# GreatV/oar-ocr

Hardware: AMD Instinct MI355X
Metric: images/sec end-to-end PP-OCRv6 det+rec (higher is better)
Workload: dtype f32; 1 GPU; PP-OCRv6-tiny-class det+rec (synthetic-weight graphs: det 447089 params, rec 1135700 params, V=6906), batch=32 synthetic 960x960 pages per GPU, 40 text lines/page; timed region = u8 pages in pageable HOST memory -> oar_ocr_predict -> oar_ocr_decode -> sorted boxes + texts + scores on the host; image_batch_size=32, region_batch_size=256, parallelism=image-parallel x1

## Files before the change

oar_ocr_amd/build.py:

```python
from __future__ import annotations

import os
import subprocess
import sys
from concurrent.futures import ThreadPoolExecutor
from pathlib import Path

HERE = Path(__file__).resolve().parent
CSRC = HERE / "csrc"
LIBDIR = HERE / "lib"
LIB = LIBDIR / "libOarMi355x.so"
SOURCES = ["common.cc", "onnx_parse.cc", "engine.cc", "db_host.cc", "poly_host.cc", "pipeline.cc", "c_api.cc", "ctc_host.cc", "image_decode.cc", "image_misc_decode.cc", "jpeg_decode.cc", "layout.cc", "kernels.hip", "igemm.hip", "igemm_ws_1x1.hip", "igemm_ws_gen.hip", "igemm_ws_x6.hip", "igemm_os_x6.hip", "igemm_ws3.hip", "igemm_rs3_x6.hip", "prepost.hip", "contours.hip", "jpeg.hip", "layout.hip", "dsblock.hip", "dsblock_k3s1.hip", "dsblock_k3s2.hip", "dsblock_k5s1.hip", "dsblock_k5s2.hip", "dsblock_wa_a.hip", "dsblock_wa_b.hip", "dsblock_rs_k3s11.hip", "dsblock_rs_k3s21.hip", "dsblock_rs_k3s12.hip", "dsblock_rs_k3s22.hip", "dsblock_rs_dbg.hip", "dsblock_cs.hip", "dsblock_pc.hip", "dsblock_rs2.hip", "ctc_head_x6.hip", "chain.hip", "attention_x6.hip", "igemm_lk_x6.hip", "index_ops.hip", "sla_decode.hip", "formula_decode.hip", "window_attention.hip", "deformable_attention.hip", "relpos_attention.hip", "mha_attention.hip", "add_layernorm.hip"]
HIPCC = os.environ.get("HIPCC", "/opt/rocm/bin/hipcc")
FLAGS = ["--offload-arch=gfx950", "-O3", "-std=c++17", "-fPIC", "-ffp-contract=off", "-fno-fast-math",
         "-Wno-unused-result", "-Wno-pass-failed"]
if os.environ.get("OAR_DSB_ABLATIONS"):
    FLAGS.append("-DOAR_DSB_ABLATIONS")


def _stale(out: Path, deps) -> bool:
    if not out.exists():
        return True
    t = out.stat().st_mtime
    return any(Path(d).stat().st_mtime > t for d in deps)


def build_lib(force: bool = False, verbose: bool = False) -> Path:
    LIBDIR.mkdir(exist_ok=True)
    objdir = LIBDIR / "obj"
    objdir.mkdir(exist_ok=True)
    headers = list(CSRC.glob("*.h")) + list(CSRC.glob("*.inc")) + [HERE.parent / "include" / "oar_mi355x.h"]
    jobs = []
    for s in SOURCES:
        src = CSRC / s
        obj = objdir / (s.replace(".", "_") + ".o")
# ... 38 lines not shown
```

oar_ocr_amd/csrc/engine.cc:

```cpp
#include "engine.h"

#include "dsblock.h"

#include <algorithm>
#include <cmath>
#include <cstring>
#include <set>
#include <sstream>

namespace oar {

using k::Act;

static int64_t numel(const std::vector<int64_t>& d) {
    int64_t n = 1;
    for (auto v : d) n *= v;
    return n;
}

Engine::Engine(const uint8_t* onnx, size_t len, int device_id, hipStream_t caller_stream) : device_(device_id) {
    int ndev = 0;
    if (hipGetDeviceCount(&ndev) != hipSuccess || ndev <= 0)
        fail(OAR_DEVICE, "no HIP device visible: libOarMi355x has no CPU fallback");
    OAR_CHECK(device_id >= 0 && device_id < ndev, OAR_DEVICE, "device_id out of range");
// ... 2705 lines not shown
        auto it = E.dev_consts_.find(key);
        if (it != E.dev_consts_.end()) return it->second;
        int64_t K = transB ? B.dims[1] : B.dims[0], N = transB ? B.dims[0] : B.dims[1];
        std::vector<float> w((size_t)N * K, 0.f);
        for (int64_t kk = 0; kk < K; ++kk)
            for (int64_t nn = 0; nn < N; ++nn) w[(size_t)nn * K + kk] = transB ? B.f[nn * K + kk] : B.f[kk * N + nn];
        return E.upload_const(key, to_fragments(fmt, w, N, K));
    }

    void get_pads(const GNode& n, int64_t H, int64_t W, int64_t kh, int64_t kw, int64_t sh, int64_t sw, int64_t dh, int64_t dw,
                  int64_t& pt, int64_t& pl, int64_t& pb, int64_t& pr) {
        std::vector<int64_t> pads = n.ais("pads");
        pt = pl = pb = pr = 0;
        if (pads.size() == 4) { pt = pads[0]; pl = pads[1]; pb = pads[2]; pr = pads[3]; }
        std::string ap = n.as("auto_pad", "NOTSET");
        if (ap == "SAME_UPPER" || ap == "SAME_LOWER") {
            int64_t oh = (H + sh - 1) / sh, ow = (W + sw - 1) / sw;
            int64_t th = std::max<int64_t>((oh - 1) * sh + (kh - 1) * dh + 1 - H, 0), tw = std::max<int64_t>((ow - 1) * sw + (kw - 1) * dw + 1 - W, 0);
            if (ap == "SAME_UPPER") { pt = th / 2; pb = th - pt; pl = tw / 2; pr = tw - pl; }
            else { pb = th / 2; pt = th - pb; pr = tw / 2; pl = tw - pr; }
        }
    }

    void op_conv(const GNode& n) {
        if (n.in.size() > 3 && !n.in[3].empty()) {
            TInfo xg = get(n.in[0]), gt = get(n.in[3]);
            const TInfo& wg = get(n.in[1]);
            bool ok = xg.dims.size() == 4 && !xg.host_int && !gt.host_int && wg.ht && wg.ht->dims.size() == 4 && gt.loc.kind != Loc::NONE && n.residual.empty();
            if (ok) {
                const int64_t N = xg.dims[0], C = xg.dims[1], HW = xg.dims[2] * xg.dims[3];
                ok = numel(gt.dims) == N * C && gt.dims.size() >= 2 && gt.dims[0] == N && gt.dims[1] == C && wg.ht->dims[1] == C && C % 8 == 0 &&
                     k::conv_igemm_se_ok(N * HW, (int)C, (int)wg.ht->dims[0], (int)HW);
            }
            if (!ok) {
                GNode mul;
                mul.op = "Mul"; mul.in = {n.in[0], n.in[3]}; mul.out = {n.out[0] + "::se"};
                op_binary(mul, 2);
                GNode c2 = n;
                c2.in.resize(3);
                c2.in[0] = mul.out[0];
                op_conv(c2);
                return;
            }
        }
        PendingConcat msrc;
        {
// ... 24 lines not shown
        int64_t pt, pl, pb, pr;
        get_pads(n, H, Wd, kh, kw, sh, sw, dh, dw, pt, pl, pb, pr);
        int64_t Ho = (H + pt + pb - dh * (kh - 1) - 1) / sh + 1, Wo = (Wd + pl + pr - dw * (kw - 1) - 1) / sw + 1;
        if (x.u8_stem) {
            OAR_CHECK(g == 1 && Cin == 3 && kh * kw * 3 <= 128 && n.residual.empty(), OAR_INTERNAL, "run_stem on a graph whose first node is not an RGB stem");
            const float* sb = has_input(n, 2) ? get(n.in[2]).loc.cptr : nullptr;
            TInfo& ys = new_out(n.out[0], {N, Cout, Ho, Wo}, Layout::CLAST);
            k::ConvP sp{};
            sp.N = (int)N; sp.H = (int)H; sp.W = (int)Wd; sp.Cin = 3; sp.Ho = (int)Ho; sp.Wo = (int)Wo; sp.Cout = (int)Cout;
            sp.kh = (int)kh; sp.kw = (int)kw; sp.sh = (int)sh; sp.sw = (int)sw; sp.pt = (int)pt; sp.pl = (int)pl; sp.dh = (int)dh; sp.dw = (int)dw;
            sp.groups = 1; sp.act = n.act; sp.bias = sb; sp.y_ld = (int)Cout; sp.convt2x2 = 0;
            sp.w = conv_weight_direct(n, W);
            const Loc ysl = ys.loc;
            step([=](const RunCtx& c) {
                OAR_CHECK(c.stem != nullptr, OAR_INTERNAL, "stem plan run without pages");
                k::ConvP q = sp;
                q.y = c.mut(ysl);
                k::conv_smallcin_u8(c.s, q, *c.stem);
            }, 2.0 * N * Ho * Wo * Cout * 3 * kh * kw, 3.0 * N * H * Wd + 4.0 * N * Ho * Wo * Cout);
            return;
        }
        Loc xin = msrc.src.empty() ? to_clast_loc(x) : Loc();
        const float* bias = has_input(n, 2) ? get(n.in[2]).loc.cptr : nullptr;
        Loc res;
        int res_up = 0;
        if (!n.residual.empty()) {
            const char* up_env = getenv("OAR_FUSE_RES_UP");
            const bool up_on = !up_env || atoi(up_env) != 0;
            if (const PendingResize* pr = peek_pending(n.residual)) {
                const bool f32_tile = g == 1 && Cin % 4 == 0 && Cout % 4 == 0 &&
                                      k::igemm_weight_format((long)(N * Ho * Wo), (int)(kh * kw * Cin), (int)Cout, kh == 1 && kw == 1 && sh == 1 && sw == 1 && pt == 0 && pl == 0, (int)Cin) == k::IGEMM_W_K16;
                if (up_on && f32_tile && pr->fh > 1 && pr->fh == pr->fw && pr->N == N && pr->C == Cout && pr->Ho == Ho && pr->Wo == Wo && Ho % pr->fh == 0 && Wo % pr->fw == 0 &&
                    pr->H * pr->fh == Ho && pr->W * pr->fw == Wo && N * Ho * Wo < ((int64_t)1 << 31)) {
                    res = pr->xin;
                    res_up = pr->fh;
                    pending_resize.erase(n.residual);
                }
            }
        }
        if (!n.residual.empty() && res_up == 0) {
            TInfo r = get(n.residual);
            if (r.host_int || r.dims != std::vector<int64_t>{N, Cout, Ho, Wo}) {
                GNode pre = n;
                pre.residual.clear();
                pre.out[0] = n.out[0] + "::pre";
                op_conv(pre);
// ... 2642 lines not shown
```

oar_ocr_amd/csrc/igemm.hip:

```cpp
#include "igemm_dev.h"

namespace oar {
namespace k {

template <int NT, int PF, bool IS1X1>
__global__ __launch_bounds__(256, 2) void conv_igemm_kernel(IgemmP p) {
    const int lane = threadIdx.x & 63, wave = threadIdx.x >> 6;
    const int pl_ = lane & 15, g = lane >> 4;
    const long b = blockIdx.x;
    const int xcd = (int)(b & 7);
    const long slot = b >> 3;
    const int ntile = (int)(slot % p.ny);
    const long mtile = (long)xcd * p.mx_per_xcd + slot / p.ny;
    if (slot / p.ny >= p.mx_per_xcd) return;
    const long m0 = (mtile * 4 + wave) * (PF * 16);
    const int nf0 = ntile * NT;
    if (m0 >= p.M) return;

    long pix_base[PF];
    int ih0[PF], iw0[PF];
#pragma unroll
    for (int pf = 0; pf < PF; ++pf) {
        long m = min(m0 + pf * 16 + pl_, p.M - 1);
        if (IS1X1) {
// ... 205 lines not shown
    const int nfrag = (N + 15) / 16, KC = (K + 15) / 16;
    int NT = 1, best = 1 << 30;
    for (int t = 4; t >= 1; --t) { int padded = (nfrag + t - 1) / t * t; if (padded < best) { best = padded; NT = t; } }
    const long ny = (nfrag + NT - 1) / NT;
    const long wave_tile_passes = ((M + 15) / 16) * ((nfrag + 7) / 8);
    const bool ws_auto = (N >= ws_min_n && wave_tile_passes >= 4096) || (K >= 512 && M >= 262144);
    const bool ws = (N & 3) == 0 && KC >= 2 && ws_mode != 0 && (ws_mode == 1 || ws_auto);
    return !ws && ((M + 15) / 16) * ny <= small_max;
}
bool conv_igemm_se_ok(long M, int K, int N, int hw) {
    static const bool on = [] { const char* e = getenv("OAR_FUSE_SE_SCALE"); return !e || atoi(e) != 0; }();
    if (!on || hw <= 0) return false;
    if (igemm_weight_format(M, K, N, true) == IGEMM_W_K16) {
        const char* e = getenv("OAR_FUSE_SE_SCALE_SMALL");
        const bool small_se = !(e && e[0] == '0');
        return small_se && (K & 3) == 0 && (N & 3) == 0 && f32_1x1_goes_small(M, K, N);
    }
    if (igemm_weight_format(M, K, N, true) != IGEMM_W_X6) return false;
    const int nfrag = (N + 15) / 16, nt = ws_x6_tile(K, nfrag);
    if (nt == 0 || os_mode() == 2) return false;
    const int ny = (nfrag + nt - 1) / nt;
    const size_t lds = (size_t)nt * ((K + 31) / 32) * 3072 + (size_t)nt * 64 + 16 + (size_t)ws_x6_se_rows(M, ny, hw) * K * 4;
    return lds <= 160 * 1024;
}

void conv_igemm(hipStream_t s, const ConvP& c) {
    IgemmP p;
    p.x = c.x; p.w = c.w; p.bias = c.bias; p.res = c.residual; p.y = c.y;
    p.H = c.H; p.W = c.W; p.Cin = c.Cin; p.kh = c.kh; p.kw = c.kw; p.sh = c.sh; p.sw = c.sw;
    p.pt = c.pt; p.pl = c.pl; p.dh = c.dh; p.dw = c.dw; p.y_ld = c.y_ld;
    p.act = c.act.kind; p.alpha = c.act.alpha; p.beta = c.act.beta;
    p.convt = c.convt2x2; p.Cout = c.Cout;
    p.ctc_part = c.ctc_part; p.ctc_valid = c.ctc_valid;
    p.se = c.se; p.se_hw = c.Ho * c.Wo;
    p.x_ld = c.x_ld > 0 ? c.x_ld : c.Cin; p.accum = c.accum;
    p.n_msrc = c.n_msrc;
    for (int i = 0; i < 8; ++i) { p.msrc[i] = i < c.n_msrc ? c.msrc[i] : nullptr; p.msrc_c[i] = i < c.n_msrc ? c.msrc_c[i] : 0; }
    p.res_up = c.residual ? c.res_up : 0;
    if (c.convt2x2) {
        p.Ho = c.H; p.Wo = c.W;
        p.M = (long)c.N * c.H * c.W; p.K = c.Cin; p.gemm_cout = 4 * c.Cout;
    } else {
        p.Ho = c.Ho; p.Wo = c.Wo;
        p.M = (long)c.N * c.Ho * c.Wo; p.K = c.kh * c.kw * c.Cin; p.gemm_cout = c.Cout;
    }
    const bool x6 = c.w_fmt == IGEMM_W_X6;
// ... 134 lines not shown
```

oar_ocr_amd/csrc/igemm_dev.h:

```cpp
#pragma once
#include <hip/hip_runtime.h>

#include <algorithm>
#include <cstdio>
#include <cstdlib>
#include <type_traits>
#include <vector>

#include "common.h"
#include "kernels_dev.h"

namespace oar {
namespace k {

struct IgemmP {
    const float* x;
    const float* w;
    const float* bias;
    const float* res;
    float* y;
    long M;
    int K, KC;
    int gemm_cout;
    int Cout;
// ... 169 lines not shown
        float4* dst = reinterpret_cast<float4*>(p.ctc_part) + row * ny + ntile;
        *dst = make_float4(m, sum, __int_as_float(last), 0.f);
    }
}

template <int NT, int PF>
__device__ __forceinline__ bool igemm_init_acc(const IgemmP& p, f32x4 (&acc)[NT][PF], int g, int nf0) {
    const bool fast = p.bias != nullptr && ((p.Cout & 3) == 0) && ((p.y_ld & 3) == 0);
#pragma clang loop unroll(full)
    for (int nf = 0; nf < NT; ++nf) {
        float4 b = make_float4(0.f, 0.f, 0.f, 0.f);
        if (fast) {
            const int c = (nf0 + nf) * 16 + g * 4;
            const int cc = c < p.gemm_cout ? c : 0;
            const int co = p.convt ? cc % p.Cout : cc;
            b = *reinterpret_cast<const float4*>(p.bias + co);
        }
#pragma clang loop unroll(full)
        for (int pf = 0; pf < PF; ++pf) acc[nf][pf] = (f32x4){b.x, b.y, b.z, b.w};
    }
    return fast;
}

void conv_igemm_ws_1x1(hipStream_t s, const IgemmP& p, int ws_nt, int ny, size_t lds);
void conv_igemm_ws_gen(hipStream_t s, const IgemmP& p, int ws_nt, int ny, size_t lds);
void conv_igemm_ws_x6(hipStream_t s, const IgemmP& p, int ws_nt, int ny, size_t lds);
int igemm_os_x6_tile(int nfrag);
void conv_igemm_os_x6(hipStream_t s, const IgemmP& p, int nfrag, bool is1x1);
bool conv_igemm_ws3_eligible(const IgemmP& p, int nfrag);
void conv_igemm_ws3(hipStream_t s, const IgemmP& p, int nfrag);
bool conv3x3_n16_x6_eligible(long M, int Cin, int Cout, long img_px, int y_ld);
std::vector<int> conv3x3_n16_x6_slices(long M, int Cin, int Cout, long img_px, int y_ld);
void conv_lk_x6(hipStream_t s, const IgemmP& p, int n_images);
void conv3x3_n16_x6(hipStream_t s, const IgemmP& p, int n_images);

}
}
```

oar_ocr_amd/csrc/igemm_ws_x6.hip:

```cpp
#include "igemm_dev.h"

namespace oar {
namespace k {

typedef __bf16 bf16x8 __attribute__((ext_vector_type(8)));

struct IgemmWsX6P {
    IgemmP g;
    int ny;
    int groups;
    long wt_per_xcd;
    long wt_total;
    int se_cap;
};

__device__ __forceinline__ void split3(const f32x4& a, const f32x4& b, uint4& h, uint4& m, uint4& l) {
    const float f[8] = {a[0], a[1], a[2], a[3], b[0], b[1], b[2], b[3]};
    unsigned hh[8], mm[8], ll[8];
#pragma clang loop unroll(full)
    for (int e = 0; e < 8; ++e) {
        const unsigned u = __float_as_uint(f[e]);
        const unsigned uh = u & 0xFFFF0000u;
        const float r1 = f[e] - __uint_as_float(uh);
        const unsigned um = __float_as_uint(r1) & 0xFFFF0000u;
        const float r2 = r1 - __uint_as_float(um);
        hh[e] = uh; mm[e] = um; ll[e] = __float_as_uint(r2) & 0xFFFF0000u;
    }
    h = make_uint4((hh[0] >> 16) | hh[1], (hh[2] >> 16) | hh[3], (hh[4] >> 16) | hh[5], (hh[6] >> 16) | hh[7]);
    m = make_uint4((mm[0] >> 16) | mm[1], (mm[2] >> 16) | mm[3], (mm[4] >> 16) | mm[5], (mm[6] >> 16) | mm[7]);
    l = make_uint4((ll[0] >> 16) | ll[1], (ll[2] >> 16) | ll[3], (ll[4] >> 16) | ll[5], (ll[6] >> 16) | ll[7]);
}

template <int NT, bool CTC = false, bool SE = false, int PF = 1>
__global__ __launch_bounds__(PF == 2 ? 512 : 1024) void conv_igemm_ws_x6_kernel(IgemmWsX6P q) {
    extern __shared__ uint4 wx_lds[];
    const IgemmP& p = q.g;
    const int lane = threadIdx.x & 63;
    const int pl_ = lane & 15, g = lane >> 4;
    const int xcd = (int)(blockIdx.x & 7);
    const int j = (int)(blockIdx.x >> 3);
    const int per_xcd = (int)(gridDim.x >> 3);
    const int team = j % q.groups, member = j / q.groups, team_size = (per_xcd - team + q.groups - 1) / q.groups;
    float* lds_bias = reinterpret_cast<float*>(wx_lds + (long)NT * p.KC * 3 * 64);
    unsigned* ws_ctr = reinterpret_cast<unsigned*>(lds_bias + NT * 16);
    float* se_lds = reinterpret_cast<float*>(ws_ctr + 4);
    long wt_begin, wt_count;
    {
        const long x0 = (long)xcd * q.wt_per_xcd, x1 = min(q.wt_total, x0 + q.wt_per_xcd);
        const long n_x = max(0L, x1 - x0), share = (n_x + team_size - 1) / team_size;
        wt_begin = x0 + (long)member * share;
        wt_count = max(0L, min(share, x1 - wt_begin));
    }
    int se_first = 0;
    if (SE && wt_count > 0) {
// ... 169 lines not shown
            m0 = m0n; u = un;
#pragma clang loop unroll(full)
            for (int pf = 0; pf < PF; ++pf) cur_row[pf] = nxt_row[pf];
        }
        asm volatile("s_waitcnt vmcnt(0)" ::: "memory");
        tie(s0); tie(s1); tie(s2);
    }
}

static int ws_x6_se_rows_pf(long M, int ny, int hw, int pf) {
    const int per_xcd = 32;
    const long wt_total = (M + 16 * pf - 1) / (16 * pf), wt_per_xcd = (wt_total + 7) / 8;
    const int groups = ny < per_xcd ? ny : per_xcd, team_min = per_xcd / groups;
    const long share = (wt_per_xcd + team_min - 1) / team_min;
    return (int)((share * 16 * pf + hw - 1) / hw) + 1;
}
static int ws_x6_pf(long M, bool ctc, int act) {
    static const int force = [] { const char* e = getenv("OAR_WS_X6_PF"); return e ? atoi(e) : 0; }();
    if (ctc) return 1;
    if (force == 1 || force == 2) return force;
    const bool cheap = act == ACT_NONE || act == ACT_RELU || act == ACT_HSWISH || act == ACT_HSIGMOID || act == ACT_LEAKY || act == ACT_CLIP;
    return (cheap && M >= 98304) ? 2 : 1;
}
int ws_x6_se_rows(long M, int ny, int hw) { return std::max(ws_x6_se_rows_pf(M, ny, hw, 1), ws_x6_se_rows_pf(M, ny, hw, 2)); }

template <int NT, bool CTC = false, bool SE = false, int PF = 1>
static void launch_ws_x6(hipStream_t s, const IgemmP& p, int ny, size_t lds) {
    OAR_MAX_LDS_ONCE((conv_igemm_ws_x6_kernel<NT, CTC, SE, PF>), 160 * 1024);
    IgemmWsX6P q;
    q.g = p; q.ny = ny;
    const int per_xcd = 32;
    q.wt_total = (p.M + 16 * PF - 1) / (16 * PF);
    q.wt_per_xcd = (q.wt_total + 7) / 8;
    q.groups = ny < per_xcd ? ny : per_xcd;
    q.se_cap = 0;
    if (SE) {
        q.se_cap = ws_x6_se_rows_pf(p.M, ny, p.se_hw, PF);
        lds += (size_t)q.se_cap * p.K * 4;
        OAR_CHECK(lds <= 160 * 1024, OAR_INTERNAL, "conv_igemm_ws_x6: the gate rows do not fit LDS (conv_igemm_se_ok should have said no)");
    }
    hipLaunchKernelGGL((conv_igemm_ws_x6_kernel<NT, CTC, SE, PF>), dim3(per_xcd * 8), dim3(PF == 2 ? 512 : 1024), lds, s, q);
}

void conv_igemm_ws_x6(hipStream_t s, const IgemmP& p, int ws_nt, int ny, size_t lds) {
    if (p.ctc_part) { launch_ws_x6<8, true>(s, p, ny, lds); return; }
    const bool two = ws_x6_pf(p.M, false, p.act) == 2;
// ... 18 lines not shown
```

oar_ocr_amd/csrc/kernels.h:

```cpp
#pragma once
#include <hip/hip_runtime.h>

#include <cstdint>
#include <vector>

namespace oar {
namespace k {

enum ActKind : int { ACT_NONE = 0, ACT_RELU, ACT_HSWISH, ACT_HSIGMOID, ACT_SIGMOID, ACT_SWISH, ACT_LEAKY, ACT_CLIP, ACT_TANH, ACT_GELU_ERF,
                     ACT_ERF, ACT_SQRT, ACT_EXP, ACT_ABS, ACT_NEG, ACT_RECIP, ACT_LOG, ACT_GELU_TANH, ACT_SOFTPLUS, ACT_FLOOR, ACT_CEIL, ACT_ROUND, ACT_NOT };
struct Act {
    int kind = ACT_NONE;
    float alpha = 0.f, beta = 0.f;
};

struct ConvP {
    int N, H, W, Cin;
    int Ho, Wo, Cout;
    int kh, kw, sh, sw, pt, pl, dh, dw, groups;
    Act act;
    const float* x;
    const float* w;
    const float* bias;
    const float* residual;
// ... 1 lines not shown
    int y_ld;
    int convt2x2;
    int w_fmt;
    float* ctc_part;
    int ctc_valid;
    const float* se;
    int res_up;
    int n_msrc;
    const float* msrc[8];
    int msrc_c[8];
    int accum;
    int x_ld;
    float* gap_part;
};
enum : int { IGEMM_W_K16 = 0, IGEMM_W_X6 = 1, IGEMM_W_X6RS = 2, IGEMM_W_X6CS = 3 };

void conv_igemm(hipStream_t s, const ConvP& p);
int igemm_weight_format(long M, int K, int N, bool is1x1, int Cin = 0, long same3x3_px = 0, bool lk_ok = false);
bool conv_lk_x6_eligible(int kh, int kw, int sh, int sw, int pt, int pl, int dh, int dw, int H, int W, int Ho, int Wo, int Cin, int Cout, int y_ld, long M);
bool conv_grouped_x6_ok(long M, int K, int N, int Cin);
bool conv_msrc_ok(long M, int K, int N);
std::vector<int> conv3x3_n16_slices(long M, int Cin, int Cout, long img_px, int y_ld);
bool conv_igemm_se_ok(long M, int K, int N, int hw);
void conv_dw(hipStream_t s, const ConvP& p);
int conv_dw_gap_tiles(const ConvP& p);
void global_avgpool_finish(hipStream_t s, const float* part, float* y, int N, int tiles, int C, int hw);
void conv_direct(hipStream_t s, const ConvP& p);
struct StemImg { const uint8_t* ptr; int32_t w; int32_t pad; };
struct StemU8 { const uint8_t* pages[32]; int src[3]; float alpha[3], beta[3]; const StemImg* dev = nullptr; };
void conv_smallcin_u8(hipStream_t s, const ConvP& p, const StemU8& st);
struct ConvT2Pair {
    const float* x; float* y;
    const float *w1, *b1, *w2, *b2;
    int N, H, W, C0, C1, C2;
    Act act1, act2;
};
bool convt2x2_pair_supported(int C0, int C1, int C2);
void convt2x2_pair(hipStream_t s, const ConvT2Pair& p);
void convt_direct(hipStream_t s, const ConvP& p);

struct PoolP {
    int N, H, W, C, Ho, Wo, kh, kw, sh, sw, pt, pl;
    int pb, pr;
    int is_max, count_include_pad;
    const float* x;
    float* y;
// ... 197 lines not shown
```

oar_ocr_amd/csrc/pipeline.cc:

```cpp
#include "pipeline.h"

#include <algorithm>
#include <map>
#include <string>
#include <cmath>
#include <chrono>
#include <cstdlib>
#include <cstring>
#include <sched.h>

namespace oar {

namespace {
struct PhaseTimer {
    bool on;
    std::chrono::steady_clock::time_point t0;
    std::vector<std::pair<const char*, double>> marks;
    PhaseTimer() {
        static const bool en = [] { const char* e = getenv("OAR_TIMING"); return e && (e[0] == '1' || e[0] == '2'); }();
        on = en;
        t0 = std::chrono::steady_clock::now();
    }
    void mark(const char* name) {
        if (!on) return;
// ... 1197 lines not shown
        for (auto& c : b) { ws.push_back(c.w); hs.push_back(c.h); }
        std::vector<int32_t> rws;
        Wts[bi] = host::rec_tensor_width(ws, hs, img_h, img_w, (int)cfg_.max_img_w, rws);
        const Plan& probe = eng_->plan_for({(int64_t)b.size(), 3, img_h, Wts[bi]}, true, false, nullptr, fuse_stem);
        OAR_CHECK(!probe.outputs.empty(), OAR_INTERNAL, "CRNN: no output returned from inference");
        fuse_tail[bi] = probe.outputs[0].dims.size() == 3 && probe.outputs[0].dims[2] > 1024;
        const Plan& plan = fuse_tail[bi] ? eng_->plan_for({(int64_t)b.size(), 3, img_h, Wts[bi]}, true, true, nullptr, fuse_stem) : probe;
        const PlanOutput& po = plan.outputs[0];
        OAR_CHECK(po.dims.size() == 3, OAR_SHAPE_MISMATCH, "CRNN: expected 3D output (batch, time, vocab)");
        OAR_CHECK(po.dims[0] == (int64_t)b.size(), OAR_SHAPE_MISMATCH, "CRNN: output batch differs from input batch");
        outs[bi].T = (uint32_t)po.dims[1]; outs[bi].V = (uint32_t)po.dims[2]; outs[bi].Wt = (uint32_t)Wts[bi];
        pend[bi].row0 = row_total; pend[bi].rows = (size_t)b.size() * po.dims[1];
        if (po.dims[2] == 0) pend[bi].rows = 0;
        row_total += pend[bi].rows;
    }
    if (row_total * 8 > idx_dev_.cap || row_total * 4 > prob_dev_.cap) {
        OAR_HIP(hipStreamSynchronize(s));
        idx_dev_.reserve(row_total * 8); prob_dev_.reserve(row_total * 4);
    }
    idx_host_.reserve(row_total * 8); prob_host_.reserve(row_total * 4);
    const int n_lanes = 1 + (int)lanes_.size();
    std::vector<char> lane_used(n_lanes, 0);
    int next_lane = 0;
    for (size_t bi = 0; bi < batches.size(); ++bi) {
        const auto& b = batches[bi];
        if (b.empty()) continue;
        const int lane = next_lane;
        next_lane = (next_lane + 1) % n_lanes;
        lane_used[lane] = 1;
        Engine& eng = lane_engine(lane);
        hipStream_t sl = eng.stream();
        int Wt = 0;
        const float* in = nullptr;
        const pp::ResizedImg* imgs = nullptr;
        if (fuse_stem) imgs = pack_u8(b, Wt, desc_slot, stage_slot, lane);
        else in = pack(b, Wt, false, desc_slot, stage_slot, lane);
        desc_slot += b.size();
        for (auto& c : b) if (!c.dev) stage_slot += ((size_t)c.w * c.h * 3 + 63) & ~(size_t)63;
        k::StemU8 st{};
        if (fuse_stem) {
            st.src[0] = 2; st.src[1] = 1; st.src[2] = 0;
            st.dev = reinterpret_cast<const k::StemImg*>(imgs);
        }
        const Plan& plan = fuse_stem ? eng.run_stem(st, {(int64_t)b.size(), 3, img_h, Wt}, fuse_tail[bi] != 0)
                                     : eng.run(in, {(int64_t)b.size(), 3, img_h, Wt}, true, fuse_tail[bi] != 0);
        if (pend[bi].rows == 0) continue;
        const PlanOutput& po = plan.outputs[0];
        if (plan.skipped_softmax && plan.ctc_part.kind != Loc::NONE)
            k::ctc_combine(sl, eng.out_ptr(plan.ctc_part), (int64_t)pend[bi].rows, plan.ctc_tiles, idx_dev_.as<int64_t>() + pend[bi].row0,
// ... 556 lines not shown
```

Before: 2458 images/sec.

## Fuse 1x1 conv with trailing height-average pool and schedule smallest rec batch first

Adds a new kernel that computes a 1x1 pointwise conv (optionally SE-gated) via split-bf16 MFMA and reduces it directly into an AveragePool over full height and width-2 windows. This avoids writing and re-reading the full conv output. The planner only uses it behind an opt-in env var. Separately, the recognizer batch loop now moves the smallest batch to the front when several lanes exist, so lanes start work sooner. The fused kernel adds a large new code path with atomic work-stealing and its own numerics.

Result: faster. 2509 images/sec (median of 6 runs) (+2.1%).

```diff
diff --git a/oar_ocr_amd/build.py b/oar_ocr_amd/build.py
--- a/oar_ocr_amd/build.py
+++ b/oar_ocr_amd/build.py
@@ -10,7 +10,7 @@
 CSRC = HERE / "csrc"
 LIBDIR = HERE / "lib"
 LIB = LIBDIR / "libOarMi355x.so"
-SOURCES = ["common.cc", "onnx_parse.cc", "engine.cc", "db_host.cc", "poly_host.cc", "pipeline.cc", "c_api.cc", "ctc_host.cc", "image_decode.cc", "image_misc_decode.cc", "jpeg_decode.cc", "layout.cc", "kernels.hip", "igemm.hip", "igemm_ws_1x1.hip", "igemm_ws_gen.hip", "igemm_ws_x6.hip", "igemm_os_x6.hip", "igemm_ws3.hip", "igemm_rs3_x6.hip", "prepost.hip", "contours.hip", "jpeg.hip", "layout.hip", "dsblock.hip", "dsblock_k3s1.hip", "dsblock_k3s2.hip", "dsblock_k5s1.hip", "dsblock_k5s2.hip", "dsblock_wa_a.hip", "dsblock_wa_b.hip", "dsblock_rs_k3s11.hip", "dsblock_rs_k3s21.hip", "dsblock_rs_k3s12.hip", "dsblock_rs_k3s22.hip", "dsblock_rs_dbg.hip", "dsblock_cs.hip", "dsblock_pc.hip", "dsblock_rs2.hip", "ctc_head_x6.hip", "chain.hip", "attention_x6.hip", "igemm_lk_x6.hip", "index_ops.hip", "sla_decode.hip", "formula_decode.hip", "window_attention.hip", "deformable_attention.hip", "relpos_attention.hip", "mha_attention.hip", "add_layernorm.hip"]
+SOURCES = ["common.cc", "onnx_parse.cc", "engine.cc", "db_host.cc", "poly_host.cc", "pipeline.cc", "c_api.cc", "ctc_host.cc", "image_decode.cc", "image_misc_decode.cc", "jpeg_decode.cc", "layout.cc", "kernels.hip", "igemm.hip", "igemm_ws_1x1.hip", "igemm_ws_gen.hip", "igemm_ws_x6.hip", "igemm_os_x6.hip", "igemm_ws3.hip", "igemm_rs3_x6.hip", "prepost.hip", "contours.hip", "jpeg.hip", "layout.hip", "dsblock.hip", "dsblock_k3s1.hip", "dsblock_k3s2.hip", "dsblock_k5s1.hip", "dsblock_k5s2.hip", "dsblock_wa_a.hip", "dsblock_wa_b.hip", "dsblock_rs_k3s11.hip", "dsblock_rs_k3s21.hip", "dsblock_rs_k3s12.hip", "dsblock_rs_k3s22.hip", "dsblock_rs_dbg.hip", "dsblock_cs.hip", "dsblock_pc.hip", "dsblock_rs2.hip", "ctc_head_x6.hip", "chain.hip", "attention_x6.hip", "igemm_lk_x6.hip", "index_ops.hip", "sla_decode.hip", "formula_decode.hip", "window_attention.hip", "deformable_attention.hip", "relpos_attention.hip", "mha_attention.hip", "add_layernorm.hip", "se_tail.hip"]
 HIPCC = os.environ.get("HIPCC", "/opt/rocm/bin/hipcc")
 FLAGS = ["--offload-arch=gfx950", "-O3", "-std=c++17", "-fPIC", "-ffp-contract=off", "-fno-fast-math",
          "-Wno-unused-result", "-Wno-pass-failed"]
diff --git a/oar_ocr_amd/csrc/engine.cc b/oar_ocr_amd/csrc/engine.cc
--- a/oar_ocr_amd/csrc/engine.cc
+++ b/oar_ocr_amd/csrc/engine.cc
@@ -2751,6 +2751,44 @@
         }
     }
 
+    bool try_conv_pool(const GNode& n, const TInfo& x, const HostTensor& W, const Loc& xin, const float* bias) {
+        const char* fe = getenv("OAR_FUSE_SE_TAIL");
+        if (!(fe && atoi(fe) != 0) || cur + 1 >= (int)E.nodes_.size() || n.out.size() != 1 || !n.residual.empty()) return false;
+        const GNode& pn = E.nodes_[cur + 1];
+        if (pn.op != "AveragePool" || pn.in.size() != 1 || pn.in[0] != n.out[0] || pn.out.size() != 1 || pn.ai("ceil_mode", 0) != 0) return false;
+        for (auto& o : E.output_names_) if (o == n.out[0]) return false;
+        for (int j = 0; j < (int)E.nodes_.size(); ++j) {
+            const GNode& q = E.nodes_[j];
+            if (j != cur + 1) for (auto& s : q.in) if (s == n.out[0]) return false;
+            if (q.residual == n.out[0]) return false;
+        }
+        const int64_t N = x.dims[0], Cin = x.dims[1], H = x.dims[2], Wd = x.dims[3], Cout = W.dims[0];
+        auto ks = pn.ais("kernel_shape"), st = pn.ais("strides");
+        if (ks.size() != 2 || st.size() != 2 || ks[0] != H || ks[1] != 2 || st[1] != 2 || Wd < 2) return false;
+        int64_t pt, pl, pb, pr;
+        get_pads(pn, H, Wd, ks[0], ks[1], st[0], st[1], 1, 1, pt, pl, pb, pr);
+        if (pt || pl || pb || pr) return false;
+        const bool gated = has_input(n, 3);
+        if (N * H * Wd >= ((int64_t)1 << 31) || !k::conv1x1_pool_ok((int)N, (int)H, (int)Wd, (int)Cin, (int)Cout, gated, n.act.kind)) return false;
+        const int64_t T = Wd / 2;
+        Loc gate;
+        if (gated) gate = get(n.in[3]).loc;
+        TInfo& y = new_out(pn.out[0], {N, Cout, 1, T}, Layout::CLAST);
+        k::ConvP p{};
+        p.N = (int)N; p.H = (int)H; p.W = (int)Wd; p.Cin = (int)Cin; p.Ho = 1; p.Wo = (int)T; p.Cout = (int)Cout;
+        p.kh = 1; p.kw = 1; p.sh = 1; p.sw = 1; p.dh = 1; p.dw = 1; p.groups = 1; p.act = n.act; p.bias = bias; p.y_ld = (int)Cout;
+        p.w_fmt = k::IGEMM_W_X6;
+        p.w = conv_weight_igemm(n, W, p.w_fmt);
+        const Loc yl = y.loc;
+        step([=](const RunCtx& c) {
+            k::ConvP q = p;
+            q.x = c.at(xin); q.y = c.mut(yl); q.se = gated ? c.at(gate) : nullptr;
+            k::conv1x1_pool(c.s, q);
+        }, 2.0 * N * H * Wd * Cout * Cin, 4.0 * (N * H * Wd * Cin + N * T * Cout + numel(W.dims)));
+        fused_into_prev.insert(cur + 1);
+        return true;
+    }
+
     void op_conv(const GNode& n) {
         if (n.in.size() > 3 && !n.in[3].empty()) {
             TInfo xg = get(n.in[0]), gt = get(n.in[3]);
@@ -2821,6 +2859,7 @@
         }
         Loc xin = msrc.src.empty() ? to_clast_loc(x) : Loc();
         const float* bias = has_input(n, 2) ? get(n.in[2]).loc.cptr : nullptr;
+        if (msrc.src.empty() && g == 1 && kh == 1 && kw == 1 && sh == 1 && sw == 1 && pt == 0 && pl == 0 && pb == 0 && pr == 0 && try_conv_pool(n, x, W, xin, bias)) return;
         Loc res;
         int res_up = 0;
         if (!n.residual.empty()) {
diff --git a/oar_ocr_amd/csrc/igemm.hip b/oar_ocr_amd/csrc/igemm.hip
--- a/oar_ocr_amd/csrc/igemm.hip
+++ b/oar_ocr_amd/csrc/igemm.hip
@@ -251,6 +251,17 @@
     const int ny = (nfrag + nt - 1) / nt;
     const size_t lds = (size_t)nt * ((K + 31) / 32) * 3072 + (size_t)nt * 64 + 16 + (size_t)ws_x6_se_rows(M, ny, hw) * K * 4;
     return lds <= 160 * 1024;
+}
+
+int conv_igemm_ws_x6_tile(long M, int K, int N, int Cin, bool gated, int hw, int act) {
+    if ((N & 3) || igemm_weight_format(M, K, N, true, Cin) != IGEMM_W_X6) return 0;
+    const int nfrag = (N + 15) / 16, nt = ws_x6_tile(K, nfrag);
+    if (nt == 0 || os_mode() == 2) return 0;
+    if (gated) return conv_igemm_se_ok(M, K, N, hw) ? nt : 0;
+    static const bool os_wide = [] { const char* e = getenv("OAR_IGEMM_OS_WIDE"); return !e || atoi(e) != 0; }();
+    const bool cheap_act = act == ACT_NONE || act == ACT_RELU;
+    if (os_wide && os_mode() != 0 && cheap_act && K >= 320 && N >= 512 && nt <= 4 && os_x6_eligible(M, K, N, Cin)) return 0;
+    return nt;
 }
 
 void conv_igemm(hipStream_t s, const ConvP& c) {
diff --git a/oar_ocr_amd/csrc/igemm_dev.h b/oar_ocr_amd/csrc/igemm_dev.h
--- a/oar_ocr_amd/csrc/igemm_dev.h
+++ b/oar_ocr_amd/csrc/igemm_dev.h
@@ -215,6 +215,24 @@
     return fast;
 }
 
+typedef __bf16 bf16x8 __attribute__((ext_vector_type(8)));
+__device__ __forceinline__ void split3(const f32x4& a, const f32x4& b, uint4& h, uint4& m, uint4& l) {
+    const float f[8] = {a[0], a[1], a[2], a[3], b[0], b[1], b[2], b[3]};
+    unsigned hh[8], mm[8], ll[8];
+#pragma clang loop unroll(full)
+    for (int e = 0; e < 8; ++e) {
+        const unsigned u = __float_as_uint(f[e]);
+        const unsigned uh = u & 0xFFFF0000u;
+        const float r1 = f[e] - __uint_as_float(uh);
+        const unsigned um = __float_as_uint(r1) & 0xFFFF0000u;
+        const float r2 = r1 - __uint_as_float(um);
+        hh[e] = uh; mm[e] = um; ll[e] = __float_as_uint(r2) & 0xFFFF0000u;
+    }
+    h = make_uint4((hh[0] >> 16) | hh[1], (hh[2] >> 16) | hh[3], (hh[4] >> 16) | hh[5], (hh[6] >> 16) | hh[7]);
+    m = make_uint4((mm[0] >> 16) | mm[1], (mm[2] >> 16) | mm[3], (mm[4] >> 16) | mm[5], (mm[6] >> 16) | mm[7]);
+    l = make_uint4((ll[0] >> 16) | ll[1], (ll[2] >> 16) | ll[3], (ll[4] >> 16) | ll[5], (ll[6] >> 16) | ll[7]);
+}
+
 void conv_igemm_ws_1x1(hipStream_t s, const IgemmP& p, int ws_nt, int ny, size_t lds);
 void conv_igemm_ws_gen(hipStream_t s, const IgemmP& p, int ws_nt, int ny, size_t lds);
 void conv_igemm_ws_x6(hipStream_t s, const IgemmP& p, int ws_nt, int ny, size_t lds);
diff --git a/oar_ocr_amd/csrc/igemm_ws_x6.hip b/oar_ocr_amd/csrc/igemm_ws_x6.hip
--- a/oar_ocr_amd/csrc/igemm_ws_x6.hip
+++ b/oar_ocr_amd/csrc/igemm_ws_x6.hip
@@ -2,8 +2,6 @@
 
 namespace oar {
 namespace k {
-
-typedef __bf16 bf16x8 __attribute__((ext_vector_type(8)));
 
 struct IgemmWsX6P {
     IgemmP g;
@@ -13,23 +11,6 @@
     long wt_total;
     int se_cap;
 };
-
-__device__ __forceinline__ void split3(const f32x4& a, const f32x4& b, uint4& h, uint4& m, uint4& l) {
-    const float f[8] = {a[0], a[1], a[2], a[3], b[0], b[1], b[2], b[3]};
-    unsigned hh[8], mm[8], ll[8];
-#pragma clang loop unroll(full)
-    for (int e = 0; e < 8; ++e) {
-        const unsigned u = __float_as_uint(f[e]);
-        const unsigned uh = u & 0xFFFF0000u;
-        const float r1 = f[e] - __uint_as_float(uh);
-        const unsigned um = __float_as_uint(r1) & 0xFFFF0000u;
-        const float r2 = r1 - __uint_as_float(um);
-        hh[e] = uh; mm[e] = um; ll[e] = __float_as_uint(r2) & 0xFFFF0000u;
-    }
-    h = make_uint4((hh[0] >> 16) | hh[1], (hh[2] >> 16) | hh[3], (hh[4] >> 16) | hh[5], (hh[6] >> 16) | hh[7]);
-    m = make_uint4((mm[0] >> 16) | mm[1], (mm[2] >> 16) | mm[3], (mm[4] >> 16) | mm[5], (mm[6] >> 16) | mm[7]);
-    l = make_uint4((ll[0] >> 16) | ll[1], (ll[2] >> 16) | ll[3], (ll[4] >> 16) | ll[5], (ll[6] >> 16) | ll[7]);
-}
 
 template <int NT, bool CTC = false, bool SE = false, int PF = 1>
 __global__ __launch_bounds__(PF == 2 ? 512 : 1024) void conv_igemm_ws_x6_kernel(IgemmWsX6P q) {
@@ -245,6 +226,7 @@
     const bool cheap = act == ACT_NONE || act == ACT_RELU || act == ACT_HSWISH || act == ACT_HSIGMOID || act == ACT_LEAKY || act == ACT_CLIP;
     return (cheap && M >= 98304) ? 2 : 1;
 }
+int ws_x6_pixel_frags(long M, int act) { return ws_x6_pf(M, false, act); }
 int ws_x6_se_rows(long M, int ny, int hw) { return std::max(ws_x6_se_rows_pf(M, ny, hw, 1), ws_x6_se_rows_pf(M, ny, hw, 2)); }
 
 template <int NT, bool CTC = false, bool SE = false, int PF = 1>
diff --git a/oar_ocr_amd/csrc/kernels.h b/oar_ocr_amd/csrc/kernels.h
--- a/oar_ocr_amd/csrc/kernels.h
+++ b/oar_ocr_amd/csrc/kernels.h
@@ -47,6 +47,8 @@
 bool conv_msrc_ok(long M, int K, int N);
 std::vector<int> conv3x3_n16_slices(long M, int Cin, int Cout, long img_px, int y_ld);
 bool conv_igemm_se_ok(long M, int K, int N, int hw);
+bool conv1x1_pool_ok(int N, int H, int W, int Cin, int Cout, bool gated, int act);
+void conv1x1_pool(hipStream_t s, const ConvP& p);
 void conv_dw(hipStream_t s, const ConvP& p);
 int conv_dw_gap_tiles(const ConvP& p);
 void global_avgpool_finish(hipStream_t s, const float* part, float* y, int N, int tiles, int C, int hw);
diff --git a/oar_ocr_amd/csrc/pipeline.cc b/oar_ocr_amd/csrc/pipeline.cc
--- a/oar_ocr_amd/csrc/pipeline.cc
+++ b/oar_ocr_amd/csrc/pipeline.cc
@@ -1243,9 +1243,18 @@
     const int n_lanes = 1 + (int)lanes_.size();
     std::vector<char> lane_used(n_lanes, 0);
     int next_lane = 0;
-    for (size_t bi = 0; bi < batches.size(); ++bi) {
+    std::vector<size_t> order;
+    for (size_t bi = 0; bi < batches.size(); ++bi) if (!batches[bi].empty()) order.push_back(bi);
+    {
+        const char* e = getenv("OAR_REC_SHORT_FIRST");
+        if (!(e && atoi(e) == 0) && n_lanes > 1 && order.size() > 2) {
+            size_t best = 0;
+            for (size_t i = 1; i < order.size(); ++i) if (batches[order[i]].size() < batches[order[best]].size()) best = i;
+            std::rotate(order.begin(), order.begin() + (ptrdiff_t)best, order.begin() + (ptrdiff_t)best + 1);
+        }
+    }
+    for (size_t bi : order) {
         const auto& b = batches[bi];
-        if (b.empty()) continue;
         const int lane = next_lane;
         next_lane = (next_lane + 1) % n_lanes;
         lane_used[lane] = 1;
diff --git a/oar_ocr_amd/csrc/se_tail.hip b/oar_ocr_amd/csrc/se_tail.hip
--- /dev/null
+++ b/oar_ocr_amd/csrc/se_tail.hip
@@ -0,0 +1,324 @@
+#include "igemm_dev.h"
+
+namespace oar {
+namespace k {
+
+int conv_igemm_ws_x6_tile(long M, int K, int N, int Cin, bool gated, int hw, int act);
+int ws_x6_pixel_frags(long M, int act);
+
+namespace {
+
+struct PwPoolP {
+    IgemmP g;
+    int ny;
+    int groups;
+    long wt_per_xcd;
+    long wt_total;
+    int se_cap;
+    int cb;
+    int T;
+};
+
+constexpr int kPoolThreads = 512;
+
+template <int NT, bool SE, int PF>
+__global__ __launch_bounds__(kPoolThreads) void conv1x1_pool_x6_kernel(PwPoolP q) {
+    extern __shared__ uint4 wx_lds[];
+    const IgemmP& p = q.g;
+    const int lane = threadIdx.x & 63;
+    const int pl_ = lane & 15, g = lane >> 4;
+    const int xcd = (int)(blockIdx.x & 7);
+    const int j = (int)(blockIdx.x >> 3);
+    const int per_xcd = (int)(gridDim.x >> 3);
+    const int team = j % q.groups, member = j / q.groups, team_size = (per_xcd - team + q.groups - 1) / q.groups;
+    float* lds_bias = reinterpret_cast<float*>(wx_lds + (long)NT * p.KC * 3 * 64);
+    unsigned* ws_ctr = reinterpret_cast<unsigned*>(lds_bias + NT * 16);
+    float* se_lds = reinterpret_cast<float*>(ws_ctr + 4);
+    long wt_begin, wt_count;
+    {
+        const long x0 = (long)xcd * q.wt_per_xcd, x1 = min(q.wt_total, x0 + q.wt_per_xcd);
+        const long n_x = max(0L, x1 - x0), share = (n_x + team_size - 1) / team_size;
+        wt_begin = x0 + (long)member * share;
+        wt_count = max(0L, min(share, x1 - wt_begin));
+    }
+    int se_first = 0;
+    if (SE && wt_count > 0) {
+        se_first = (int)(wt_begin / q.cb);
+        const int se_last = (int)((wt_begin + wt_count - 1) / q.cb);
+        if (se_last - se_first + 1 > q.se_cap) __builtin_trap();
+        const int cnt = (se_last - se_first + 1) * p.K;
+        for (int i = threadIdx.x; i < cnt; i += blockDim.x) se_lds[i] = p.se[(long)se_first * p.K + i];
+    }
+    const int cols = 2 * q.T;
+    constexpr int NL = 2 * PF;
+    auto issue = [](f32x4& dst, const float* src) { asm volatile("global_load_dwordx4 %0, %1, off" : "=v"(dst) : "v"(src)); };
+    struct Stage { f32x4 a[PF], b[PF]; };
+    auto tie = [](Stage& st) {
+        if constexpr (PF == 1) asm volatile("" : "+v"(st.a[0]), "+v"(st.b[0]));
+        else asm volatile("" : "+v"(st.a[0]), "+v"(st.b[0]), "+v"(st.a[1]), "+v"(st.b[1]));
+    };
+    auto x_addr = [&](long row_base, int kc) -> const float* {
+        return p.x + row_base + min(kc * 32 + 8 * g, p.K - 8);
+    };
+    auto grab = [&]() -> long {
+        unsigned u = 0;
+        if (lane == 0) u = atomicAdd(ws_ctr, 1u);
+        return (long)(unsigned)__builtin_amdgcn_readfirstlane((int)u);
+    };
+    auto row_of = [&](long t, int r, int pf) -> long {
+        const long n = t / q.cb;
+        const int c = min((int)(t - n * q.cb) * 16 + pl_, cols - 1), row = min(r * PF + pf, p.H - 1);
+        return ((n * p.H + row) * (long)p.W + c) * (long)p.Cin;
+    };
+    const int passes = (p.H + PF - 1) / PF;
+    const float div = (float)(2 * p.H);
+
+    for (int ntile = team; ntile < q.ny; ntile += q.groups) {
+        const int nf0 = ntile * NT;
+        __syncthreads();
+        if (threadIdx.x == 0) *ws_ctr = 0;
+        if (threadIdx.x < NT * 16) {
+            const int c = nf0 * 16 + (int)threadIdx.x;
+            lds_bias[threadIdx.x] = (p.bias && c < p.gemm_cout) ? p.bias[c] : 0.f;
+        }
+        {
+            const uint4* wsrc = reinterpret_cast<const uint4*>(p.w) + (long)nf0 * p.KC * 3 * 64;
+            const int total = NT * p.KC * 3 * 64;
+            for (int i0 = threadIdx.x; i0 < total; i0 += (int)blockDim.x) {
+                const int r = i0 % 192, f = i0 / 192;
+                const int nf = f / p.KC, kc = f - nf * p.KC;
+                wx_lds[(kc * NT + nf) * 192 + r] = wsrc[i0];
+            }
+        }
+        __syncthreads();
+
+        long u = grab();
+        if (u >= wt_count) continue;
+        int r = 0;
+        long cur_row[PF], nxt_row[PF];
+#pragma clang loop unroll(full)
+        for (int pf = 0; pf < PF; ++pf) { cur_row[pf] = row_of(wt_begin + u, 0, pf); nxt_row[pf] = cur_row[pf]; }
+        Stage s0, s1, s2;
+        auto stage = [&](auto Ic) -> Stage& {
+            constexpr int I = decltype(Ic)::value % 3;
+            if constexpr (I == 0) return s0; else if constexpr (I == 1) return s1; else return s2;
+        };
+#pragma clang loop unroll(full)
+        for (int pf = 0; pf < PF; ++pf) { const float* a0 = x_addr(cur_row[pf], 0); issue(s0.a[pf], a0); issue(s0.b[pf], a0 + 4); }
+#pragma clang loop unroll(full)
+        for (int pf = 0; pf < PF; ++pf) { const float* a1 = x_addr(cur_row[pf], min(1, p.KC - 1)); issue(s1.a[pf], a1); issue(s1.b[pf], a1 + 4); }
+        asm volatile("s_waitcnt vmcnt(0)" ::: "memory");
+        tie(s0); tie(s1);
+
+        f32x4 ps[NT];
+#pragma clang loop unroll(full)
+        for (int nf = 0; nf < NT; ++nf) ps[nf] = (f32x4){0.f, 0.f, 0.f, 0.f};
+
+        const uint4* wl = wx_lds + lane;
+        auto run_row = [&]() {
+            const long img = (wt_begin + u) / q.cb;
+            const float* se_row = SE ? se_lds + (long)((int)img - se_first) * p.K : nullptr;
+            f32x4 acc[NT][PF];
+#pragma clang loop unroll(full)
+            for (int nf = 0; nf < NT; ++nf) {
+                const float4 bq = *reinterpret_cast<const float4*>(lds_bias + nf * 16 + g * 4);
+#pragma clang loop unroll(full)
+                for (int pf = 0; pf < PF; ++pf) acc[nf][pf] = (f32x4){bq.x, bq.y, bq.z, bq.w};
+            }
+            uint4 wr[2][3];
+#pragma clang loop unroll(full)
+            for (int pq = 0; pq < 3; ++pq) wr[0][pq] = wl[pq * 64];
+            auto chunk = [&](int kc, auto SIc, auto WAITc, auto R0c) {
+                constexpr int SI = decltype(SIc)::value, r0 = decltype(R0c)::value;
+                constexpr bool WAIT = decltype(WAITc)::value;
+                Stage& cs = stage(std::integral_constant<int, SI>{});
+                Stage& ns = stage(std::integral_constant<int, SI + 2>{});
+                if (WAIT) { asm volatile("s_waitcnt vmcnt(%0)" ::"n"(NL) : "memory"); tie(cs); }
+                {
+                    const int k2 = kc + 2;
+                    const bool in_cur = k2 < p.KC;
+#pragma clang loop unroll(full)
+                    for (int pf = 0; pf < PF; ++pf) {
+                        const float* ap = x_addr(in_cur ? cur_row[pf] : nxt_row[pf], in_cur ? k2 : k2 - p.KC);
+                        issue(ns.a[pf], ap); issue(ns.b[pf], ap + 4);
+                    }
+                }
+                uint4 xs[PF][3];
+#pragma clang loop unroll(full)
+                for (int pf = 0; pf < PF; ++pf) {
+                    if (SE) {
+                        const float* sp = se_row + min(kc * 32 + 8 * g, p.K - 8);
+                        const f32x4 ga = *reinterpret_cast<const f32x4*>(sp), gb = *reinterpret_cast<const f32x4*>(sp + 4);
+                        split3(cs.a[pf] * ga, cs.b[pf] * gb, xs[pf][0], xs[pf][1], xs[pf][2]);
+                    } else {
+                        split3(cs.a[pf], cs.b[pf], xs[pf][0], xs[pf][1], xs[pf][2]);
+                    }
+                }
+                const int k1 = min(kc + 1, p.KC - 1);
+#pragma clang loop unroll(full)
+                for (int nf = 0; nf < NT; ++nf) {
+                    {
+                        const int nf2 = (nf + 1) % NT;
+                        const int kq = (nf + 1 < NT) ? kc : k1;
+                        __builtin_amdgcn_sched_barrier(0);
+#pragma clang loop unroll(full)
+                        for (int pq = 0; pq < 3; ++pq) wr[(r0 + nf + 1) & 1][pq] = wl[(((long)kq * NT + nf2) * 3 + pq) * 64];
+                        __builtin_amdgcn_sched_barrier(0);
+                    }
+                    const uint4* w = wr[(r0 + nf) & 1];
+                    constexpr int WP[6] = {1, 2, 0, 1, 0, 0};
+                    constexpr int XP[6] = {1, 0, 2, 0, 1, 0};
+#pragma clang loop unroll(full)
+                    for (int t = 0; t < 6; ++t)
+#pragma clang loop unroll(full)
+                        for (int pf = 0; pf < PF; ++pf)
+                            acc[nf][pf] = __builtin_amdgcn_mfma_f32_16x16x32_bf16(__builtin_bit_cast(bf16x8, w[WP[t]]), __builtin_bit_cast(bf16x8, xs[pf][XP[t]]), acc[nf][pf], 0, 0, 0);
+                }
+            };
+            using I0 = std::integral_constant<int, 0>;
+            using I1 = std::integral_constant<int, 1>;
+            using I2 = std::integral_constant<int, 2>;
+            using Wy = std::true_type;
+            using Wn = std::false_type;
+            constexpr int O = NT & 1;
+            chunk(0, I0{}, Wn{}, I0{});
+            chunk(1, I1{}, Wn{}, std::integral_constant<int, O>{});
+            int kc = 2;
+            for (; kc + 5 < p.KC; kc += 6) {
+                chunk(kc, I2{}, Wy{}, I0{}); chunk(kc + 1, I0{}, Wy{}, std::integral_constant<int, O>{}); chunk(kc + 2, I1{}, Wy{}, I0{});
+                chunk(kc + 3, I2{}, Wy{}, std::integral_constant<int, O>{}); chunk(kc + 4, I0{}, Wy{}, I0{}); chunk(kc + 5, I1{}, Wy{}, std::integral_constant<int, O>{});
+            }
+            if (kc < p.KC) chunk(kc, I2{}, Wy{}, I0{});
+            if (kc + 1 < p.KC) chunk(kc + 1, I0{}, Wy{}, std::integral_constant<int, O>{});
+            if (kc + 2 < p.KC) chunk(kc + 2, I1{}, Wy{}, I0{});
+            if (kc + 3 < p.KC) chunk(kc + 3, I2{}, Wy{}, std::integral_constant<int, O>{});
+            if (kc + 4 < p.KC) chunk(kc + 4, I0{}, Wy{}, I0{});
+            asm volatile("s_waitcnt vmcnt(0)" ::: "memory");
+            tie(s0); tie(s1); tie(s2);
+            auto act_all = [&](auto f) {
+#pragma clang loop unroll(full)
+                for (int nf = 0; nf < NT; ++nf)
+#pragma clang loop unroll(full)
+                    for (int pf = 0; pf < PF; ++pf)
+#pragma clang loop unroll(full)
+                        for (int e = 0; e < 4; ++e) acc[nf][pf][e] = f(acc[nf][pf][e]);
+            };
+            switch (p.act) {
+                case ACT_NONE: break;
+                case ACT_RELU: act_all([](float v) { return !(v <= 0.f) ? v : 0.f; }); break;
+                case ACT_HSWISH: act_all([](float v) { float t = fminf(fmaxf(v * (1.0f / 6.0f) + 0.5f, 0.f), 1.f); return v * t; }); break;
+                default: { const int kind = p.act; const float al = p.alpha, be = p.beta; act_all([=](float v) { return apply_act(v, kind, al, be); }); } break;
+            }
+#pragma clang loop unroll(full)
+            for (int nf = 0; nf < NT; ++nf)
+#pragma clang loop unroll(full)
+                for (int pf = 0; pf < PF; ++pf) {
+                    f32x4 nb;
+#pragma clang loop unroll(full)
+                    for (int e = 0; e < 4; ++e) nb[e] = __shfl_down(acc[nf][pf][e], 1, 64);
+                    if (r * PF + pf < p.H) {
+                        ps[nf] += acc[nf][pf];
+                        ps[nf] += nb;
+                    }
+                }
+            if (r == passes - 1) {
+                const int col = (int)(wt_begin + u - img * q.cb) * 16 + pl_;
+#pragma clang loop unroll(full)
+                for (int nf = 0; nf < NT; ++nf) {
+                    const int ch = (nf0 + nf) * 16 + g * 4;
+                    if (!(pl_ & 1) && col < cols && ch < p.gemm_cout)
+                        *reinterpret_cast<float4*>(p.y + (img * q.T + (col >> 1)) * (long)p.y_ld + ch) = make_float4(ps[nf][0] / div, ps[nf][1] / div, ps[nf][2] / div, ps[nf][3] / div);
+                    ps[nf] = (f32x4){0.f, 0.f, 0.f, 0.f};
+                }
+            }
+        };
+
+        for (;;) {
+            long un = u;
+            int rn = r + 1;
+            bool has_next = true;
+            if (rn == passes) { rn = 0; un = grab(); has_next = un < wt_count; }
+#pragma clang loop unroll(full)
+            for (int pf = 0; pf < PF; ++pf) nxt_row[pf] = has_next ? row_of(wt_begin + un, rn, pf) : cur_row[pf];
+            run_row();
+            if (!has_next) break;
+            const int rot = p.KC % 3;
+            if (rot == 1) { s0 = s1; s1 = s2; }
+            else if (rot == 2) { s1 = s0; s0 = s2; }
+            u = un; r = rn;
+#pragma clang loop unroll(full)
+            for (int pf = 0; pf < PF; ++pf) cur_row[pf] = nxt_row[pf];
+        }
+        asm volatile("s_waitcnt vmcnt(0)" ::: "memory");
+        tie(s0); tie(s1); tie(s2);
+    }
+}
+
+constexpr int kPerXcd = 32;
+
+int pool_se_rows(long wt_total, int ny, int cb) {
+    const long wt_per_xcd = (wt_total + 7) / 8;
+    const int groups = ny < kPerXcd ? ny : kPerXcd, team_min = kPerXcd / groups;
+    const long share = (wt_per_xcd + team_min - 1) / team_min;
+    return (int)((share + cb - 1) / cb) + 1;
+}
+
+struct PoolGeom { int nt, pf, ny, cb, se_cap; size_t lds; };
+
+bool pool_geom(int N, int H, int W, int K, int Cout, bool gated, int act, PoolGeom& o) {
+    if (N <= 0 || H <= 0 || W < 2 || (K & 7) || (Cout & 15)) return false;
+    const long M = (long)N * H * W;
+    o.nt = conv_igemm_ws_x6_tile(M, K, Cout, K, gated, H * W, act);
+    const int nfrag = Cout / 16;
+    if (o.nt == 0 || (o.nt & 1) || nfrag % o.nt != 0 || (K + 31) / 32 < 2) return false;
+    o.pf = (o.nt == 4 && H >= 2 && ws_x6_pixel_frags(M, act) == 2) ? 2 : 1;
+    o.ny = nfrag / o.nt;
+    o.cb = (2 * (W / 2) + 15) / 16;
+    o.se_cap = gated ? pool_se_rows((long)N * o.cb, o.ny, o.cb) : 0;
+    o.lds = (size_t)o.nt * ((K + 31) / 32) * 3072 + (size_t)o.nt * 64 + 16 + (size_t)o.se_cap * K * 4;
+    return o.lds <= 160 * 1024 && (long)N * (W / 2) * Cout < (1L << 40);
+}
+
+template <int NT, bool SE, int PF>
+void launch_pool(hipStream_t s, const PwPoolP& q, size_t lds) {
+    OAR_MAX_LDS_ONCE((conv1x1_pool_x6_kernel<NT, SE, PF>), 160 * 1024);
+    hipLaunchKernelGGL((conv1x1_pool_x6_kernel<NT, SE, PF>), dim3(kPerXcd * 8), dim3(kPoolThreads), lds, s, q);
+}
+
+}
+
+bool conv1x1_pool_ok(int N, int H, int W, int Cin, int Cout, bool gated, int act) {
+    PoolGeom gm;
+    return pool_geom(N, H, W, Cin, Cout, gated, act, gm);
+}
+
+void conv1x1_pool(hipStream_t s, const ConvP& c) {
+    if (c.N == 0) return;
+    PoolGeom gm;
+    OAR_CHECK(c.w_fmt == IGEMM_W_X6 && !c.residual && (c.y_ld & 3) == 0 && pool_geom(c.N, c.H, c.W, c.Cin, c.Cout, c.se != nullptr, c.act.kind, gm), OAR_INTERNAL,
+              "conv1x1_pool: a layer the planner should not have fused (conv1x1_pool_ok)");
+    PwPoolP q{};
+    IgemmP& p = q.g;
+    p.x = c.x; p.w = c.w; p.bias = c.bias; p.y = c.y; p.se = c.se;
+    p.H = c.H; p.W = c.W; p.Cin = c.Cin; p.y_ld = c.y_ld;
+    p.act = c.act.kind; p.alpha = c.act.alpha; p.beta = c.act.beta;
+    p.Cout = c.Cout; p.gemm_cout = c.Cout;
+    p.M = (long)c.N * c.H * c.W; p.K = c.Cin; p.KC = (c.Cin + 31) / 32;
+    q.ny = gm.ny; q.groups = gm.ny < kPerXcd ? gm.ny : kPerXcd;
+    q.cb = gm.cb; q.T = c.W / 2;
+    q.wt_total = (long)c.N * gm.cb; q.wt_per_xcd = (q.wt_total + 7) / 8;
+    q.se_cap = gm.se_cap;
+    const double flops = 2.0 * (double)p.M * p.K * c.Cout;
+    const double bytes = 4.0 * ((double)p.M * c.Cin + (double)c.N * q.T * c.Cout + (double)p.K * c.Cout);
+    ProfScope ps(s, "conv_igemm_ws_x6_pool", bytes, flops);
+    const bool se = c.se != nullptr;
+    if (gm.pf == 2) { se ? launch_pool<4, true, 2>(s, q, gm.lds) : launch_pool<4, false, 2>(s, q, gm.lds); return; }
+    switch (gm.nt) {
+        case 8: se ? launch_pool<8, true, 1>(s, q, gm.lds) : launch_pool<8, false, 1>(s, q, gm.lds); break;
+        case 6: se ? launch_pool<6, true, 1>(s, q, gm.lds) : launch_pool<6, false, 1>(s, q, gm.lds); break;
+        default: se ? launch_pool<4, true, 1>(s, q, gm.lds) : launch_pool<4, false, 1>(s, q, gm.lds); break;
+    }
+}
+
+}
+}
```
